# tejank10/AlphaGo.jl

Measured on AMD Instinct MI355X. Metric: self-play positions/sec (9x9, tower=10, 400 readouts), higher is better.
Workload: dtype f32

## Files before the change

### alphago.jl_amd/csrc/agz_nn.h

```cpp
#pragma once
#include <algorithm>
#include <cstdint>
#include <functional>
#include <memory>
#include <type_traits>
#include <vector>

#include "agz_common.h"

namespace agz {

constexpr int kC = 256;
constexpr int kCinStem = 17;
constexpr int kCinStemPad = 32;
constexpr int kWinoStages = 64, kWinoStemStages = 8;

struct ConvHost {
  int k = 3, cin = 0, cout = 0;
  std::vector<float> w, b, beta, gamma, mean, var;
  float eps = 1e-5f;
};
struct DenseHost {
  int in = 0, out = 0;
  std::vector<float> w, b;
// ... 55 lines not shown
    if (winograd_ == 0) return TowerForm::Direct;
    if (precision_ == 0 && winograd_ != 2 && wino4_applies(N_)) return TowerForm::Wino4;
    if (precision_ == 0 && winograd_ == 3 && wino_fusable(N_)) return TowerForm::Wino5;
    return tower_persistent_ && wino_fusable(N_) ? TowerForm::Wino3Persistent : TowerForm::Wino3;
  }

  float mfma_sustained_tflops(int millis, int mode = 0);
  void profile_enable(bool on);
  void profile_read(double* total_ms, double* total_flop, int64_t* launches);

  ConvHost* conv(int layer);
  const ConvHost* conv(int layer) const;
  DenseHost* dense(int layer);
  const DenseHost* dense(int layer) const;
  void sync_host() const;
  uint64_t param_version() const { return param_version_; }

  double flops_per_eval() const;
  double conv_flops_per_launch(int B) const { return 2.0 * B * P_ * 9.0 * kC * kC; }

 private:
  void pack();
  enum ImageId { kDirectStem, kDirectTower, kWinoStem, kWinoTower, kSplitStem, kSplitTower, kWino4Tower, kWino5Tower, kF16Tower, kImages };
  struct BuiltImage {
    const ImageFamily* family;
    bool stem;
    int which;
    bool (*needed)(const Net&);
    DevBuf<uint32_t> buf;
    uint64_t version = ~0ull;
  };
  static bool always(const Net&) { return true; }
  static bool with_tower(const Net& n) { return n.tower_ > 0; }
  static bool split_selected(const Net& n) { return n.tower_ > 0 && n.precision_ == 2; }
  template <TowerForm F> static bool form_is(const Net& n) { return n.tower_form() == F; }
  BuiltImage images_[kImages] = {{&kDirectImage, true, 0, always},
                                 {&kDirectImage, false, 0, with_tower},
                                 {&kWinoImage, true, 1, with_tower},
                                 {&kWinoImage, false, 1, with_tower},
                                 {&kWinoSplitImage, true, 4, split_selected},
                                 {&kWinoSplitImage, false, 4, split_selected},
                                 {&kWino4Image, false, 2, form_is<TowerForm::Wino4>},
                                 {&kWino5Image, false, 6, form_is<TowerForm::Wino5>},
                                 {&kConv16Image, false, 3, form_is<TowerForm::F16>}};
  uint64_t affines_version_ = ~0ull;
  int image_stages(const BuiltImage& im) const { return im.stem ? kWinoStemStages : kWinoStages; }
  template <class T>
  const T* image(ImageId id, int l = 0) const {
    const BuiltImage& im = images_[id];
    return reinterpret_cast<const T*>(im.buf.p + im.family->bytes(image_stages(im)) / 4 * l);
  }
  void stem(TowerForm form, const float* d_x32, const int* d_count, int bcap);
  void direct_tower(const int* d_count, int bcap);
  void f16_tower(const int* d_count, int bcap);
  void wino_tower(TowerForm form, const int* d_count, int bcap);
  void persistent_tower(const int* d_count, int bcap);
  struct LayerIO { const float *vin, *res; float *y, *vout; };
  LayerIO layer_io(int l, bool dense) const;
  void wino_layer(TowerForm form, int l, const LayerIO& io, const int* d_count, int bcap, hipStream_t st, int part = 0,
                  int parts = 1);
  template <class Layer> void run_chains(int chains, const Layer& layer);
  template <class Launch> void timed(int layers, const Launch& launch);

  int N_, P_, A_, tower_;
  hipStream_t stream_;
  ConvHost stem_, vconv_, pconv_;
  std::vector<ConvHost> tconv_;
  DenseHost vfc1_, vfc2_, pfc_;
  struct FluxSlot { int layer, kind; size_t off, n; };
  std::vector<FluxSlot> slots_;
  size_t flux_n_ = 0;
  DevBuf<float> d_flux_;
  mutable bool host_stale_ = false;
  uint64_t param_version_ = 0;
  void upload_slot(const FluxSlot& s);
  void upload_host_all();
  const float* host_slot(const FluxSlot& s) const;

  DevBuf<float> d_scale_, d_shift_;
  DevBuf<float> d_head_;
  const float *d_vfc1w_ = nullptr, *d_vfc1b_ = nullptr, *d_vfc2w_ = nullptr, *d_vfc2b_ = nullptr, *d_pfcw_ = nullptr,
              *d_pfcb_ = nullptr;
  int bcap_ = 0;
  DevBuf<float> d_a_, d_b_, d_t_, d_vh_, d_ph_;
  int winograd_ = 1;
  static constexpr int kMaxTowerStreams = 4;
  int tower_streams_ = 2;
  hipStream_t streamx_[kMaxTowerStreams - 1] = {nullptr, nullptr, nullptr};
  hipEvent_t ev_fork_ = nullptr, ev_join_[kMaxTowerStreams - 1] = {nullptr, nullptr, nullptr};
  DevBuf<float> d_scale_s_;
  DevBuf<float> d_vimg_, d_vimg2_;
  int precision_ = 0;
  DevBuf<uint16_t> d_ha_, d_hb_, d_ht_;
  bool tower_persistent_ = false;
  DevBuf<int> d_tower_sched_;
  DevBuf<char> d_tower_layers_;
  std::vector<char> tower_layers_host_;
  int32_t* tower_err_ = nullptr;
  std::vector<int> prof_mult_;
  bool prof_on_ = false;
  std::vector<hipEvent_t> prof_ev_;
  std::vector<int> prof_fwd_of_;
  int32_t* prof_counts_ = nullptr;
  int prof_n_ = 0, prof_fwd_ = 0;
  static constexpr int kProfMax = 4096;
};

class Trainer {
 public:
  Trainer(Net& net, hipStream_t s);
  ~Trainer();
  void step(const float* feats, const float* pi, const float* z, int B, bool is_device, float eta, float rho,
            float* losses_out);
  void reset();

 private:
  struct Param;
  void upload();
  void publish(long M);
  uint64_t uploaded_version_ = ~0ull;
  Net& net_;
  hipStream_t stream_;
  std::vector<std::unique_ptr<Param>> params_;
  bool have_vel_ = false;
  DevBuf<float> d_x32_, d_u_, d_o_, d_ga_, d_gb_, d_gc_, d_stats_, d_ones_, d_zero_, d_wd_, d_small_, d_in_, d_part_, d_wpart_;
  DevBuf<double> d_sums_;
  DevBuf<int> d_cnt_;
  DevBuf<unsigned char> d_opta_, d_optw_;
  int n_optw_ = 0;
};

void launch_conv3x3_direct_taps(const float* x, const float* wt, const float* ones, const float* zeros, const float* shift,
                                float* y, float* part, const int* d_count, int bcap, int N, int cin_pad, hipStream_t s);
int conv3x3_direct_blocks(int bcap, int N);
void launch_conv3x3_direct(const float* x, const float* wt, const float* scale, const float* shift, const float* res,
                           float* y, const int* d_count, int bcap, int N, int relu, int cin_pad, hipStream_t s);

size_t wino_v_floats(int bcap, int T);
long wino_blocks(int bcap, int T);
inline void wino_block_range(int blocks, int part, int parts, bool pairs, int& tb0, int& tb1) {
  AGZ_REQUIRE(parts >= 1 && part >= 0 && part < parts, AGZ_BAD_ARGUMENT, "tile-block range %d of %d", part, parts);
  int per = (blocks + parts - 1) / parts;
  if (pairs) per = (per + 1) & ~1;
  tb0 = std::min(blocks, part * per);
  tb1 = part + 1 == parts ? blocks : std::min(blocks, tb0 + per);
}
inline void wino_check_32bit(long blocks, int rows, int bcap, int N) {
  AGZ_REQUIRE((blocks + 1) * rows < (1L << 31) && (long)bcap * N * N * kC * 4 < (1L << 32), AGZ_BAD_ARGUMENT,
              "batch of %d positions at %dx%d: tile index / activation byte offset exceeds 32 bits", bcap, N, N);
}
void launch_wino_in(const float* x, float* vimg, const int* d_count, int bcap, int N, bool split, hipStream_t s,
                    int ns = kWinoStages, bool fixup = false);
void launch_wino_gemm(const float* vimg, const float* uimg, const float* scale, const float* shift, const float* res,
                      float* y, float* vnext, const int* d_count, int bcap, int N, int relu, bool split, hipStream_t s,
                      int ns = kWinoStages, int part = 0, int parts = 1);
bool wino_fusable(int N);
struct WinoTowerLayer {
  const float *v, *u, *scale, *shift, *res;
  float *y, *vnext;
  int mode, relu;
};
size_t wino_tower_sched_ints(int layers, int bcap, int N);
bool wino_tower_supported(hipStream_t s);
void launch_wino_tower(const void* d_layers, int layers, int* d_sched, const int* d_count, int bcap, int N, bool split, hipStream_t s);
constexpr int kWinoTowerErrWord = 8;
float wino_split_descale();

// ... 39 lines not shown
```

### alphago.jl_amd/csrc/agz_nn.hip

```cpp
#include "agz_nn.h"
#include "agz_pack.h"

#include <cmath>
#include <algorithm>
#include <cstring>

#include "../../include/agz_draws.h"

namespace agz {

typedef float f32x16 __attribute__((ext_vector_type(16)));


constexpr int BM = 128, BN = 128, BK = 32;
constexpr int LDS_STRIDE = BK + 4;

template <int CIN, bool TAPSPLIT = false>
__global__ __launch_bounds__(256, 2) void k_conv3x3_mfma(
    const float* __restrict__ x, const float* __restrict__ wt, const float* __restrict__ scale,
    const float* __restrict__ shift, const float* __restrict__ res, float* __restrict__ y,
    const int* __restrict__ d_count, int N, int relu, long ystride = 0) {
  constexpr int NCHUNK = 9 * CIN / BK;
  constexpr int CPT = CIN / BK;
  const int c_begin = TAPSPLIT ? (int)blockIdx.y * CPT : 0, c_end = TAPSPLIT ? c_begin + CPT : NCHUNK;
// ... 35 lines not shown
    const int tap_ = (c) / CPT, ci0_ = ((c) % CPT) * BK;          \
    const int da_ = tap_ % 3 - 1, db_ = tap_ / 3 - 1;             \
    const int aoff_ = ci0_ + c4 * 4, boff_ = (c) * BK;            \
    AGZ_LOADROW(0, da_, db_, aoff_, boff_)                        \
    AGZ_LOADROW(1, da_, db_, aoff_, boff_)                        \
    AGZ_LOADROW(2, da_, db_, aoff_, boff_)                        \
    AGZ_LOADROW(3, da_, db_, aoff_, boff_)                        \
  }
#define AGZ_STOREROW(buf, i)                                                                           \
  *reinterpret_cast<float4*>(&lds[buf][0][(lrow + 32 * i) * LDS_STRIDE + c4 * 4]) = ra##i;             \
  *reinterpret_cast<float4*>(&lds[buf][1][(lrow + 32 * i) * LDS_STRIDE + c4 * 4]) = rb##i;
#define AGZ_STORE_CHUNK(buf) { AGZ_STOREROW(buf, 0) AGZ_STOREROW(buf, 1) AGZ_STOREROW(buf, 2) AGZ_STOREROW(buf, 3) }

  const int lane = tid & 63, wave = tid >> 6;
  const int wr = wave >> 1, wc = wave & 1;
  const int l31 = lane & 31, hi = lane >> 5;

  f32x16 acc[2][2];
#pragma unroll
  for (int a = 0; a < 2; ++a)
#pragma unroll
    for (int b = 0; b < 2; ++b)
#pragma unroll
      for (int e = 0; e < 16; ++e) acc[a][b][e] = 0.f;

  AGZ_LOAD_CHUNK(c_begin)
  AGZ_STORE_CHUNK(0)
  __syncthreads();

  for (int c = c_begin; c < c_end; ++c) {
    const int buf = (c - c_begin) & 1;
    if (c + 1 < c_end) AGZ_LOAD_CHUNK(c + 1)
    const float* As = &lds[buf][0][(wr * 64 + l31) * LDS_STRIDE + hi * 4];
    const float* Bs = &lds[buf][1][(wc * 64 + l31) * LDS_STRIDE + hi * 4];
#pragma unroll
    for (int kk = 0; kk < BK / 8; ++kk) {
      const float4 a0 = *reinterpret_cast<const float4*>(As + kk * 8);
      const float4 a1 = *reinterpret_cast<const float4*>(As + 32 * LDS_STRIDE + kk * 8);
      const float4 b0 = *reinterpret_cast<const float4*>(Bs + kk * 8);
      const float4 b1 = *reinterpret_cast<const float4*>(Bs + 32 * LDS_STRIDE + kk * 8);
#define AGZ_MFMA4(f)                                                                          \
  acc[0][0] = __builtin_amdgcn_mfma_f32_32x32x2f32(a0.f, b0.f, acc[0][0], 0, 0, 0);             \
  acc[0][1] = __builtin_amdgcn_mfma_f32_32x32x2f32(a0.f, b1.f, acc[0][1], 0, 0, 0);             \
  acc[1][0] = __builtin_amdgcn_mfma_f32_32x32x2f32(a1.f, b0.f, acc[1][0], 0, 0, 0);             \
  acc[1][1] = __builtin_amdgcn_mfma_f32_32x32x2f32(a1.f, b1.f, acc[1][1], 0, 0, 0);
      AGZ_MFMA4(x) AGZ_MFMA4(y) AGZ_MFMA4(z) AGZ_MFMA4(w)
#undef AGZ_MFMA4
    }
    if (c + 1 < c_end) AGZ_STORE_CHUNK(buf ^ 1)
    __syncthreads();
  }

#undef AGZ_LOADROW
#undef AGZ_LOAD_CHUNK
#undef AGZ_STOREROW
#undef AGZ_STORE_CHUNK
#pragma unroll
  for (int tn = 0; tn < 2; ++tn) {
    const int n = n0 + wc * 64 + tn * 32 + l31;
    const float sc = scale[n], sh = shift[n];
#pragma unroll
    for (int tm = 0; tm < 2; ++tm) {
#pragma unroll
      for (int e = 0; e < 16; ++e) {
        const long m = m0 + wr * 64 + tm * 32 + (e & 3) + 8 * (e >> 2) + 4 * hi;
        if (m < M) {
          float v = acc[tm][tn][e] * sc + sh;
          if (res) v += res[m * kC + n];
          if (relu) v = fmaxf(v, 0.f);
          y[m * kC + n] = v;
        }
      }
    }
  }
}


__device__ __forceinline__ float wave_sum(float v) {
#pragma unroll
  for (int o = 32; o > 0; o >>= 1) v += __shfl_xor(v, o, 64);
  return v;
}

__global__ __launch_bounds__(256) void k_head_conv(const float* __restrict__ x, const float* __restrict__ hp,
                                                    float* __restrict__ vh, float* __restrict__ ph,
                                                    const int* __restrict__ d_count, int P) {
  const long M = (long)(*d_count) * P;
  const int lane = threadIdx.x & 63, wave = threadIdx.x >> 6;
  const float4 wv = *reinterpret_cast<const float4*>(hp + lane * 4);
  const float4 w0 = *reinterpret_cast<const float4*>(hp + 256 + lane * 4);
  const float4 w1 = *reinterpret_cast<const float4*>(hp + 512 + lane * 4);
  const float sv = hp[768], tv = hp[769], s0 = hp[770], t0 = hp[771], s1 = hp[772], t1 = hp[773];
  for (long m = (long)blockIdx.x * 4 + wave; m < M; m += (long)gridDim.x * 4) {
    const float4 xv = *reinterpret_cast<const float4*>(x + m * kC + lane * 4);
    float dv = xv.x * wv.x + xv.y * wv.y + xv.z * wv.z + xv.w * wv.w;
    float d0 = xv.x * w0.x + xv.y * w0.y + xv.z * w0.z + xv.w * w0.w;
    float d1 = xv.x * w1.x + xv.y * w1.y + xv.z * w1.z + xv.w * w1.w;
    dv = wave_sum(dv);
    d0 = wave_sum(d0);
    d1 = wave_sum(d1);
    if (lane == 0) {
      vh[m] = fmaxf(dv * sv + tv, 0.f);
      ph[m * 2 + 0] = fmaxf(d0 * s0 + t0, 0.f);
      ph[m * 2 + 1] = fmaxf(d1 * s1 + t1, 0.f);
    }
  }
}

__device__ float block_reduce(float v, bool is_max, float* red ) {
  const int lane = threadIdx.x & 63, wave = threadIdx.x >> 6;
#pragma unroll
  for (int o = 32; o > 0; o >>= 1) {
    const float t = __shfl_xor(v, o, 64);
    v = is_max ? fmaxf(v, t) : v + t;
  }
  __syncthreads();
  if (lane == 0) red[wave] = v;
  __syncthreads();
  float r = red[0];
#pragma unroll
  for (int w = 1; w < 4; ++w) r = is_max ? fmaxf(r, red[w]) : r + red[w];
  return r;
}

__global__ __launch_bounds__(256) void k_head_fc(
    const float* __restrict__ vh, const float* __restrict__ ph, const float* __restrict__ w1,
    const float* __restrict__ b1, const float* __restrict__ w2, const float* __restrict__ b2,
    const float* __restrict__ wp, const float* __restrict__ bp, float* __restrict__ pi,
    float* __restrict__ v, const int* __restrict__ d_count, int P, int A) {
  extern __shared__ __attribute__((aligned(16))) float sm[];
  float* vin = sm;
  float* pin = sm + P;
  float* logit = pin + 2 * P;
  float* red = logit + A;
  const int b = blockIdx.x;
  if (b >= *d_count) return;
  const int tid = threadIdx.x;
  for (int i = tid; i < P; i += 256) {
    vin[i] = vh[(long)b * P + i];
    pin[i] = ph[((long)b * P + i) * 2 + 0];
    pin[P + i] = ph[((long)b * P + i) * 2 + 1];
  }
  __syncthreads();
  float lmax = -INFINITY;
  for (int o = tid; o < A; o += 256) {
    float z = bp[o];
    for (int i = 0; i < 2 * P; ++i) z += wp[o + (long)A * i] * pin[i];
    logit[o] = z;
    lmax = fmaxf(lmax, z);
  }
  const float mx = block_reduce(lmax, true, red);
  float lsum = 0.f;
  for (int o = tid; o < A; o += 256) {
    const float e = expf(logit[o] - mx);
    logit[o] = e;
    lsum += e;
  }
  const float sum = block_reduce(lsum, false, red);
  for (int o = tid; o < A; o += 256) pi[(long)b * A + o] = logit[o] / sum;
  float h = b1[tid];
  for (int i = 0; i < P; ++i) h += w1[tid + 256 * i] * vin[i];
  h = fmaxf(h, 0.f);
  const float s = block_reduce(h * w2[tid], false, red);
  if (tid == 0) v[b] = tanhf(s + b2[0]);
}


__global__ __launch_bounds__(128) void k_feats_from_deltas(
    const int8_t* __restrict__ boards, const int8_t* __restrict__ deltas, const int32_t* __restrict__ ndeltas,
    const int8_t* __restrict__ to_play, int B, int N, float* __restrict__ x32, float* __restrict__ whcn) {
  const int b = blockIdx.x;
  if (b >= B) return;
  const int P = N * N;
  const int nd = ndeltas[b];
  const int tp = to_play[b];
  for (int p = threadIdx.x; p < P; p += blockDim.x) {
    int cur = boards[(long)b * P + p];
    float f[32];
#pragma unroll
    for (int k = 0; k < 8; ++k) {
      if (k >= 1 && k <= nd) cur -= deltas[((long)b * 7 + (k - 1)) * P + p];
      f[2 * k] = cur == tp ? 1.f : 0.f;
      f[2 * k + 1] = cur == -tp ? 1.f : 0.f;
    }
    f[16] = (float)tp;
#pragma unroll
    for (int c = 17; c < 32; ++c) f[c] = 0.f;
    if (x32) {
      float4* dst = reinterpret_cast<float4*>(x32 + ((long)b * P + p) * 32);
#pragma unroll
      for (int c = 0; c < 8; ++c) dst[c] = make_float4(f[4 * c], f[4 * c + 1], f[4 * c + 2], f[4 * c + 3]);
    }
    if (whcn) {
#pragma unroll
      for (int c = 0; c < 17; ++c) whcn[(long)P * (c + 17L * b) + p] = f[c];
    }
  }
}

__global__ __launch_bounds__(128) void k_whcn_to_x32(const float* __restrict__ whcn, int B, int P,
                                                      float* __restrict__ x32) {
  const int b = blockIdx.x;
  if (b >= B) return;
  for (int p = threadIdx.x; p < P; p += blockDim.x) {
    float* dst = x32 + ((long)b * P + p) * 32;
    for (int c = 0; c < 17; ++c) dst[c] = whcn[(long)P * (c + 17L * b) + p];
    for (int c = 17; c < 32; ++c) dst[c] = 0.f;
  }
}

void launch_features_from_deltas(const int8_t* d_boards, const int8_t* d_deltas, const int32_t* d_ndeltas,
                                 const int8_t* d_to_play, int B, int N, float* d_x32, float* d_whcn,
                                 hipStream_t stream) {
  if (B <= 0) return;
  hipLaunchKernelGGL(k_feats_from_deltas, dim3(B), dim3(128), 0, stream, d_boards, d_deltas, d_ndeltas,
                     d_to_play, B, N, d_x32, d_whcn);
  AGZ_HIP(hipGetLastError());
}

void launch_whcn_to_x32(const float* d_whcn, int B, int N, float* d_x32, hipStream_t stream) {
  if (B <= 0) return;
  hipLaunchKernelGGL(k_whcn_to_x32, dim3(B), dim3(128), 0, stream, d_whcn, B, N * N, d_x32);
  AGZ_HIP(hipGetLastError());
}


static void conv_init(ConvHost& c, int k, int cin, int cout) {
  c.k = k; c.cin = cin; c.cout = cout;
  c.w.assign((size_t)k * k * cin * cout, 0.f);
  c.b.assign(cout, 0.f);
  c.beta.assign(cout, 0.f);
  c.gamma.assign(cout, 1.f);
  c.mean.assign(cout, 0.f);
  c.var.assign(cout, 1.f);
  c.eps = 1e-5f;
}
static void dense_init(DenseHost& d, int in, int out) {
  d.in = in; d.out = out;
  d.w.assign((size_t)in * out, 0.f);
  d.b.assign(out, 0.f);
}

static std::vector<float>* conv_field(ConvHost* c, int kind);

Net::Net(int N, int tower, hipStream_t stream) : N_(N), P_(N * N), A_(N * N + 1), tower_(tower), stream_(stream) {
  conv_init(stem_, 3, kCinStem, kC);
  tconv_.resize(2 * tower);
// ... 236 lines not shown
    launched = true;
  }
  if (affines_version_ != param_version_) {
    d_scale_.ensure((size_t)L * kC);
    d_shift_.ensure((size_t)L * kC);
    d_scale_s_.ensure((size_t)L * kC);
    hipLaunchKernelGGL(k_bn_affine, dim3(1), dim3(256), 0, stream_, F + flux_offset(0, AGZ_K_BIAS), 0L, 1, kC, d_scale_.p, d_shift_.p,
                       d_scale_s_.p + (size_t)2 * tower_ * kC, wino_split_descale());
    if (tower_ > 0)
      hipLaunchKernelGGL(k_bn_affine, dim3(2 * tower_), dim3(256), 0, stream_, F + flux_offset(1, AGZ_K_BIAS), tstride(), 2 * tower_, kC,
                         d_scale_.p + kC, d_shift_.p + kC, d_scale_s_.p, wino_split_descale());
    d_head_.ensure(776);
    hipLaunchKernelGGL(k_pack_head, dim3(1), dim3(256), 0, stream_, F + flux_offset(AGZ_L_VALUE_CONV, AGZ_K_WEIGHT),
                       F + flux_offset(AGZ_L_POLICY_CONV, AGZ_K_WEIGHT), d_head_.p);
    d_vfc1w_ = F + flux_offset(AGZ_L_VALUE_FC1, AGZ_K_WEIGHT); d_vfc1b_ = F + flux_offset(AGZ_L_VALUE_FC1, AGZ_K_BIAS);
    d_vfc2w_ = F + flux_offset(AGZ_L_VALUE_FC2, AGZ_K_WEIGHT); d_vfc2b_ = F + flux_offset(AGZ_L_VALUE_FC2, AGZ_K_BIAS);
    d_pfcw_ = F + flux_offset(AGZ_L_POLICY_FC, AGZ_K_WEIGHT); d_pfcb_ = F + flux_offset(AGZ_L_POLICY_FC, AGZ_K_BIAS);
    affines_version_ = param_version_;
    launched = true;
  }
  if (launched) AGZ_HIP(hipGetLastError());
}

long Net::debug_pack_diff(int which) {
  pack();
  sync_host();
  if (which < 0 || which > 6) return -1;
  const int L = 1 + 2 * tower_;
  auto diff = [&](const auto* dev, const auto& host) {
    static_assert(sizeof(host[0]) == 4, "debug_pack_diff counts 32-bit words");
    auto got = host;
    download(got.data(), dev, got.size(), stream_);
    AGZ_HIP(hipStreamSynchronize(stream_));
    long bad = 0;
    for (size_t i = 0; i < got.size(); ++i) bad += std::memcmp(&got[i], &host[i], 4) != 0;
    return bad;
  };
  long bad = 0;
  for (const BuiltImage& im : images_) {
    if (im.which != which || !im.needed(*this)) continue;
    std::vector<uint32_t> img(im.family->bytes(image_stages(im)) / 4);
    for (int l = 0; l < (im.stem ? 1 : 2 * tower_); ++l) {
      im.family->host_pack(im.stem ? stem_ : tconv_[l], img.data(), image_stages(im));
      bad += diff(im.buf.p + img.size() * l, img);
    }
  }
  if (which == 4 && images_[kSplitTower].needed(*this)) {
    std::vector<float> sc((size_t)L * kC), tmp(kC);
    for (int l = 0; l <= 2 * tower_; ++l) {
      bn_affine(l < 2 * tower_ ? tconv_[l] : stem_, sc.data() + (size_t)l * kC, tmp.data());
      for (int o = 0; o < kC; ++o) sc[(size_t)l * kC + o] *= wino_split_descale();
    }
    bad += diff(d_scale_s_.p, sc);
  }
  if (which == 5) {
    std::vector<float> scale((size_t)L * kC), shift((size_t)L * kC);
    bn_affine(stem_, scale.data(), shift.data());
    for (int l = 0; l < 2 * tower_; ++l) bn_affine(tconv_[l], scale.data() + (size_t)(l + 1) * kC, shift.data() + (size_t)(l + 1) * kC);
    bad += diff(d_scale_.p, scale) + diff(d_shift_.p, shift);
    std::vector<float> hp(776, 0.f);
    for (int c = 0; c < kC; ++c) { hp[c] = vconv_.w[c]; hp[256 + c] = pconv_.w[c]; hp[512 + c] = pconv_.w[kC + c]; }
    float s[2], t[2];
    bn_affine(vconv_, s, t);
    hp[768] = s[0]; hp[769] = t[0];
    bn_affine(pconv_, s, t);
    hp[770] = s[0]; hp[771] = t[0]; hp[772] = s[1]; hp[773] = t[1];
    bad += diff(d_head_.p, hp);
  }
  return bad;
}

void Net::reserve(int bcap) {
  if (precision_ == 1 && tower_ > 0 && d_ha_.n < ((size_t)std::max(bcap, bcap_) * P_ + 256) * kC) {
    const size_t n = ((size_t)std::max(bcap, bcap_) * P_ + 256) * kC;
    d_ha_.alloc(n);
    d_hb_.alloc(n);
    d_ht_.alloc(n);
  }
  if (bcap <= bcap_) return;
  const size_t rows = (size_t)bcap * P_;
  d_a_.alloc(rows * kC);
  d_b_.alloc(rows * kC);
  d_t_.alloc(rows * kC);
  d_vh_.alloc(rows);
  d_ph_.alloc(rows * 2);
  if (tower_ > 0) {
    const size_t vf = std::max(wino_v_floats(bcap, (N_ + 2) / 3), wino4_applies(N_) ? wino4_v_floats(bcap, N_) : (size_t)0);
    d_vimg_.alloc(vf);
    d_vimg2_.alloc(vf);
  }
  bcap_ = bcap;
}

static inline int conv_grid(int bcap, int P) { return ceil_div((long)bcap * P, BM) * (kC / BN); }
int conv3x3_direct_blocks(int bcap, int N) { return conv_grid(bcap, N * N); }

void launch_conv3x3_direct(const float* x, const float* wt, const float* scale, const float* shift, const float* res,
                           float* y, const int* d_count, int bcap, int N, int relu, int cin_pad, hipStream_t s) {
  const int grid = conv_grid(bcap, N * N);
  if (cin_pad == kCinStemPad)
    hipLaunchKernelGGL((k_conv3x3_mfma<kCinStemPad>), dim3(grid), dim3(256), 0, s, x, wt, scale, shift, res, y, d_count, N, relu);
  else
    hipLaunchKernelGGL((k_conv3x3_mfma<kC>), dim3(grid), dim3(256), 0, s, x, wt, scale, shift, res, y, d_count, N, relu);
}

__global__ __launch_bounds__(256) void k_sum_taps(const float* __restrict__ part, long stride, const float* __restrict__ shift,
                                                   float* __restrict__ y, const int* __restrict__ d_count, int P) {
  const long n4 = (long)(*d_count) * P * (kC / 4);
  for (long i = (long)blockIdx.x * 256 + threadIdx.x; i < n4; i += (long)gridDim.x * 256) {
    float4 s = *reinterpret_cast<const float4*>(part + i * 4);
#pragma unroll
    for (int z = 1; z < 9; ++z) {
      const float4 v = *reinterpret_cast<const float4*>(part + z * stride + i * 4);
      s.x += v.x; s.y += v.y; s.z += v.z; s.w += v.w;
    }
    const float4 b = *reinterpret_cast<const float4*>(shift + (i * 4) % kC);
    *reinterpret_cast<float4*>(y + i * 4) = make_float4(s.x + b.x, s.y + b.y, s.z + b.z, s.w + b.w);
  }
}

void launch_conv3x3_direct_taps(const float* x, const float* wt, const float* ones, const float* zeros, const float* shift,
                                float* y, float* part, const int* d_count, int bcap, int N, int cin_pad, hipStream_t s) {
  const int grid = conv_grid(bcap, N * N);
  const long stride = (long)bcap * N * N * kC;
  if (cin_pad == kCinStemPad)
    hipLaunchKernelGGL((k_conv3x3_mfma<kCinStemPad, true>), dim3(grid, 9), dim3(256), 0, s, x, wt, ones, zeros,
                       (const float*)nullptr, part, d_count, N, 0, stride);
  else
    hipLaunchKernelGGL((k_conv3x3_mfma<kC, true>), dim3(grid, 9), dim3(256), 0, s, x, wt, ones, zeros, (const float*)nullptr,
                       part, d_count, N, 0, stride);
  const int g = (int)std::min<long>(((long)bcap * N * N * (kC / 4) + 255) / 256, 2048);
  hipLaunchKernelGGL(k_sum_taps, dim3(g), dim3(256), 0, s, (const float*)part, stride, shift, y, d_count, N * N);
}

template <class Launch> void Net::timed(int layers, const Launch& launch) {
  const bool p = prof_on_ && prof_n_ < kProfMax;
  if (p) (void)hipEventRecord(prof_ev_[2 * prof_n_], stream_);
  launch();
  if (p) {
    (void)hipEventRecord(prof_ev_[2 * prof_n_ + 1], stream_);
    prof_mult_[prof_n_] = layers;
    prof_fwd_of_[prof_n_++] = prof_fwd_;
  }
}

template <class Layer> void Net::run_chains(int chains, const Layer& layer) {
  const int nl = 2 * tower_;
  if (chains == 1) {
    for (int l = 0; l < nl; ++l) timed(1, [&] { layer(l, 0, stream_); });
    return;
  }
  if (!ev_fork_) AGZ_HIP(hipEventCreateWithFlags(&ev_fork_, hipEventDisableTiming));
  for (int i = 0; i + 1 < chains; ++i)
    if (!streamx_[i]) {
      AGZ_HIP(hipStreamCreateWithFlags(&streamx_[i], hipStreamNonBlocking));
      AGZ_HIP(hipEventCreateWithFlags(&ev_join_[i], hipEventDisableTiming));
    }
  auto join = [&] {
    for (int i = 0; i + 1 < chains; ++i) {
      (void)hipEventRecord(ev_join_[i], streamx_[i]);
      (void)hipStreamWaitEvent(stream_, ev_join_[i], 0);
    }
  };
  timed(nl, [&] {
    AGZ_HIP(hipEventRecord(ev_fork_, stream_));
    for (int i = 0; i + 1 < chains; ++i) AGZ_HIP(hipStreamWaitEvent(streamx_[i], ev_fork_, 0));
    try {
      for (int part = 0; part < chains; ++part)
// ... 79 lines not shown
  }
}

Net::LayerIO Net::layer_io(int l, bool dense) const {
  if (l % 2 == 0) return {d_vimg_.p, nullptr, dense ? d_t_.p : nullptr, d_vimg2_.p};
  const bool odd = (l / 2) % 2;
  return {d_vimg2_.p, odd ? d_b_.p : d_a_.p, odd ? d_a_.p : d_b_.p, l + 1 == 2 * tower_ ? nullptr : d_vimg_.p};
}

void Net::wino_layer(TowerForm form, int l, const LayerIO& io, const int* d_count, int bcap, hipStream_t st, int part, int parts) {
  const float* sc = d_scale_.p + (size_t)(l + 1) * kC;
  const float* sh = d_shift_.p + (size_t)(l + 1) * kC;
  if (form == TowerForm::Wino4) {
    launch_wino4_gemm(io.vin, image<float>(kWino4Tower, l), sc, sh, io.res, io.y, io.vout, d_count, bcap, N_, 1, st,
                      part, parts, io.y && !io.res && wino4_paired(N_));
    if (io.vout && !wino4_whole_boards(N_)) launch_wino4_in(io.y, io.vout, d_count, bcap, N_, st, true, part, parts);
  } else if (form == TowerForm::Wino5) {
    launch_wino5_gemm(io.vin, image<float>(kWino5Tower, l), sc, sh, io.res, io.y, io.vout, d_count, bcap, N_, 1, st,
                      part, parts);
  } else {
    const bool split = precision_ == 2;
    const float* u = image<float>(split ? kSplitTower : kWinoTower, l);
    launch_wino_gemm(io.vin, u, split ? d_scale_s_.p + (size_t)l * kC : sc, sh, io.res, io.y, io.vout, d_count, bcap, N_, 1, split,
                     st, kWinoStages, part, parts);
    if (io.vout && !wino_fusable(N_)) launch_wino_in(io.y, io.vout, d_count, bcap, N_, split, st, kWinoStages, true);
  }
}

void Net::wino_tower(TowerForm form, const int* d_count, int bcap) {
  const bool f44 = form == TowerForm::Wino4;
  const bool dense = f44 ? !wino4_whole_boards(N_) : !wino_fusable(N_);
  const int T = f44 ? (N_ + 3) / 4 : (N_ + 2) / 3;
  const int chains = dense && !f44 ? 1 : chain_count(tower_streams_, (long)bcap * T * T, f44 ? 64 : 63);
  run_chains(chains, [&](int l, int part, hipStream_t st) {
    wino_layer(form, l, layer_io(l, dense), d_count, bcap, st, part, chains);
  });
}

void Net::persistent_tower(const int* d_count, int bcap) {
  const bool split = precision_ == 2;
  const ImageId u = split ? kSplitTower : kWinoTower;
  const float* sc = split ? d_scale_s_.p : d_scale_.p + kC;
  const float* sh = d_shift_.p + kC;
  const int nl = 2 * tower_;
  std::vector<WinoTowerLayer> tab(nl);
  for (int l = 0; l < nl; ++l) {
    const LayerIO io = layer_io(l, false);
    tab[l] = {io.vin, image<float>(u, l), sc + (size_t)l * kC, sh + (size_t)l * kC, io.res, io.y, io.vout,
              (io.y ? 1 : 0) | (io.vout ? 2 : 0), 1};
  }
  const size_t tbytes = sizeof(WinoTowerLayer) * tab.size();
  if (tower_layers_host_.size() != tbytes || std::memcmp(tower_layers_host_.data(), tab.data(), tbytes) != 0) {
    AGZ_HIP(hipStreamSynchronize(stream_));
    tower_layers_host_.assign((const char*)tab.data(), (const char*)tab.data() + tbytes);
    d_tower_layers_.ensure(tbytes);
    AGZ_HIP(hipMemcpy(d_tower_layers_.p, tower_layers_host_.data(), tbytes, hipMemcpyHostToDevice));
  }
  d_tower_sched_.ensure(wino_tower_sched_ints(nl, bcap, N_));
  if (!tower_err_) {
    AGZ_HIP(hipHostMalloc((void**)&tower_err_, sizeof(int32_t), hipHostMallocDefault));
    *tower_err_ = 0;
  }
  timed(nl, [&] { launch_wino_tower(d_tower_layers_.p, nl, d_tower_sched_.p, d_count, bcap, N_, split, stream_); });
  (void)hipMemcpyAsync(tower_err_, d_tower_sched_.p + kWinoTowerErrWord, sizeof(int32_t), hipMemcpyDeviceToHost, stream_);
}

void Net::forward(const float* d_x32, const int* d_count, int bcap, float* d_pi, float* d_v) {
  check_async_error();
  TowerForm form = tower_form();
  if (form == TowerForm::Wino4) wino4_validate(bcap, N_);
  pack();
  reserve(bcap);
  if (prof_on_ && prof_fwd_ < kProfMax)
    (void)hipMemcpyAsync(&prof_counts_[prof_fwd_], d_count, sizeof(int32_t), hipMemcpyDeviceToHost, stream_);
  stem(form, d_x32, d_count, bcap);
  if (form == TowerForm::Wino3Persistent && !wino_tower_supported(stream_)) form = TowerForm::Wino3;
  switch (form) {
    case TowerForm::Direct: direct_tower(d_count, bcap); break;
    case TowerForm::F16: f16_tower(d_count, bcap); break;
    case TowerForm::Wino3Persistent: persistent_tower(d_count, bcap); break;
    default: wino_tower(form, d_count, bcap); break;
  }
  const float* x = form == TowerForm::F16 || tower_ % 2 ? d_b_.p : d_a_.p;
  const int hgrid = std::min(ceil_div((long)bcap * P_, 4), 256 * 16);
  hipLaunchKernelGGL(k_head_conv, dim3(hgrid), dim3(256), 0, stream_, x, d_head_.p, d_vh_.p, d_ph_.p, d_count, P_);
  const size_t smem = sizeof(float) * (size_t)(3 * P_ + A_ + 4);
  hipLaunchKernelGGL(k_head_fc, dim3(bcap), dim3(256), smem, stream_, (const float*)d_vh_.p,
                     (const float*)d_ph_.p, d_vfc1w_, d_vfc1b_, d_vfc2w_, d_vfc2b_, d_pfcw_,
                     d_pfcb_, d_pi, d_v, d_count, P_, A_);
  if (prof_on_ && prof_fwd_ < kProfMax) prof_fwd_++;
  AGZ_HIP(hipGetLastError());
}

__global__ __launch_bounds__(256) void k_mfma_f32_sustained(int iters, float* out) {
  typedef float f32x16 __attribute__((ext_vector_type(16)));
  f32x16 acc[8];
#pragma unroll
  for (int i = 0; i < 8; ++i)
#pragma unroll
    for (int e = 0; e < 16; ++e) acc[i][e] = 0.f;
  const float a = 1.f + threadIdx.x * 1e-6f, b = 0.5f;
  for (int it = 0; it < iters; ++it) {
#pragma unroll
    for (int i = 0; i < 8; ++i) acc[i] = __builtin_amdgcn_mfma_f32_32x32x2f32(a, b, acc[i], 0, 0, 0);
  }
  float s = 0.f;
#pragma unroll
  for (int i = 0; i < 8; ++i) s += acc[i][0] + acc[i][15];
  if (s == 123.456f) out[0] = s;
}

template <bool F16, bool DENSE>
__global__ __launch_bounds__(256) void k_mfma_sustained_data(int iters, float* out) {
  typedef float f32x16 __attribute__((ext_vector_type(16)));
  typedef _Float16 h8 __attribute__((ext_vector_type(8)));
  f32x16 acc[8];
#pragma unroll
  for (int i = 0; i < 8; ++i)
#pragma unroll
    for (int e = 0; e < 16; ++e) acc[i][e] = 0.f;
  unsigned st = 0x9e3779b9u * (threadIdx.x + 256u * blockIdx.x + 1u);
  auto rnd = [&]() { st = st * 1664525u + 1013904223u; return (float)(int)(st >> 8) * (1.0f / 8388608.0f) - 1.0f; };
  float a32[16], b32[16];
  h8 a16[16], b16[16];
#pragma unroll
  for (int k = 0; k < 16; ++k) {
    a32[k] = rnd(); b32[k] = DENSE ? rnd() : fmaxf(rnd(), 0.f) * 2.f;
#pragma unroll
    for (int e = 0; e < 8; ++e) {
      a16[k][e] = (_Float16)(0.06f * rnd());
      b16[k][e] = (_Float16)(DENSE ? rnd() : fmaxf(rnd(), 0.f) * 2.f);
    }
  }
  for (int it = 0; it < iters; it += 16) {
#pragma unroll
    for (int u = 0; u < 16; ++u)
#pragma unroll
      for (int i = 0; i < 8; ++i) {
        if (F16) acc[i] = __builtin_amdgcn_mfma_f32_32x32x16_f16(a16[(i + u) & 15], b16[(3 * i + 5 * u) & 15], acc[i], 0, 0, 0);
        else acc[i] = __builtin_amdgcn_mfma_f32_32x32x2f32(a32[(i + u) & 15], b32[(3 * i + 5 * u) & 15], acc[i], 0, 0, 0);
      }
  }
  float s = 0.f;
#pragma unroll
  for (int i = 0; i < 8; ++i) s += acc[i][0] + acc[i][15];
  if (s == 123.456f) out[0] = s;
}

float Net::mfma_sustained_tflops(int millis, int mode) {
  AGZ_REQUIRE(millis >= 50 && millis <= 5000, AGZ_BAD_ARGUMENT, "mfma_sustained_tflops: %d ms (50..5000)", millis);
  AGZ_REQUIRE(mode >= 0 && mode <= 4, AGZ_BAD_ARGUMENT, "mfma_sustained_tflops: mode %d", mode);
  const bool f16 = mode == 2 || mode == 4;
  DevBuf<float> out;
  out.alloc(16);
  hipEvent_t e0, e1;
  AGZ_HIP(hipEventCreate(&e0));
  AGZ_HIP(hipEventCreate(&e1));
  const int iters = f16 ? 20000 : 10000, grid = 1024;
  const double flop = (double)grid * 4 * iters * 8.0 * (f16 ? 32768.0 : 4096.0);
  std::vector<double> tf;
  double spent = 0.0;
  while (spent < millis) {
    AGZ_HIP(hipEventRecord(e0, stream_));
    if (mode == 0) hipLaunchKernelGGL(k_mfma_f32_sustained, dim3(grid), dim3(256), 0, stream_, iters, out.p);
    else if (mode == 1) hipLaunchKernelGGL((k_mfma_sustained_data<false, false>), dim3(grid), dim3(256), 0, stream_, iters, out.p);
    else if (mode == 2) hipLaunchKernelGGL((k_mfma_sustained_data<true, false>), dim3(grid), dim3(256), 0, stream_, iters, out.p);
    else if (mode == 3) hipLaunchKernelGGL((k_mfma_sustained_data<false, true>), dim3(grid), dim3(256), 0, stream_, iters, out.p);
    else hipLaunchKernelGGL((k_mfma_sustained_data<true, true>), dim3(grid), dim3(256), 0, stream_, iters, out.p);
    AGZ_HIP(hipEventRecord(e1, stream_));
    AGZ_HIP(hipEventSynchronize(e1));
    float ms = 0.f;
    AGZ_HIP(hipEventElapsedTime(&ms, e0, e1));
// ... 75 lines not shown
```

Measured before the change: 447.5.

## Fuse head conv and FC into one kernel processing eight boards per block

Merges the 1x1 head convolution and the value/policy fully connected layers into a single kernel, so the intermediate vh/ph buffers no longer go through global memory. Each block now handles eight boards, with per-board inputs interleaved in shared memory. Every weight loaded from wp and w1 is therefore reused across eight boards instead of being re-read per board. The trade-offs are fewer blocks (less parallelism for small batches), higher register pressure from the per-board arrays, and more shared memory per block.

Result: no change. 448.6, median of 3 (+0.2%).

```diff
diff --git a/alphago.jl_amd/csrc/agz_nn.h b/alphago.jl_amd/csrc/agz_nn.h
--- a/alphago.jl_amd/csrc/agz_nn.h
+++ b/alphago.jl_amd/csrc/agz_nn.h
@@ -161,7 +161,7 @@
   const float *d_vfc1w_ = nullptr, *d_vfc1b_ = nullptr, *d_vfc2w_ = nullptr, *d_vfc2b_ = nullptr, *d_pfcw_ = nullptr,
               *d_pfcb_ = nullptr;
   int bcap_ = 0;
-  DevBuf<float> d_a_, d_b_, d_t_, d_vh_, d_ph_;
+  DevBuf<float> d_a_, d_b_, d_t_;
   int winograd_ = 1;
   static constexpr int kMaxTowerStreams = 4;
   int tower_streams_ = 2;
diff --git a/alphago.jl_amd/csrc/agz_nn.hip b/alphago.jl_amd/csrc/agz_nn.hip
--- a/alphago.jl_amd/csrc/agz_nn.hip
+++ b/alphago.jl_amd/csrc/agz_nn.hip
@@ -141,31 +141,6 @@
   return v;
 }
 
-__global__ __launch_bounds__(256) void k_head_conv(const float* __restrict__ x, const float* __restrict__ hp,
-                                                    float* __restrict__ vh, float* __restrict__ ph,
-                                                    const int* __restrict__ d_count, int P) {
-  const long M = (long)(*d_count) * P;
-  const int lane = threadIdx.x & 63, wave = threadIdx.x >> 6;
-  const float4 wv = *reinterpret_cast<const float4*>(hp + lane * 4);
-  const float4 w0 = *reinterpret_cast<const float4*>(hp + 256 + lane * 4);
-  const float4 w1 = *reinterpret_cast<const float4*>(hp + 512 + lane * 4);
-  const float sv = hp[768], tv = hp[769], s0 = hp[770], t0 = hp[771], s1 = hp[772], t1 = hp[773];
-  for (long m = (long)blockIdx.x * 4 + wave; m < M; m += (long)gridDim.x * 4) {
-    const float4 xv = *reinterpret_cast<const float4*>(x + m * kC + lane * 4);
-    float dv = xv.x * wv.x + xv.y * wv.y + xv.z * wv.z + xv.w * wv.w;
-    float d0 = xv.x * w0.x + xv.y * w0.y + xv.z * w0.z + xv.w * w0.w;
-    float d1 = xv.x * w1.x + xv.y * w1.y + xv.z * w1.z + xv.w * w1.w;
-    dv = wave_sum(dv);
-    d0 = wave_sum(d0);
-    d1 = wave_sum(d1);
-    if (lane == 0) {
-      vh[m] = fmaxf(dv * sv + tv, 0.f);
-      ph[m * 2 + 0] = fmaxf(d0 * s0 + t0, 0.f);
-      ph[m * 2 + 1] = fmaxf(d1 * s1 + t1, 0.f);
-    }
-  }
-}
-
 __device__ float block_reduce(float v, bool is_max, float* red ) {
   const int lane = threadIdx.x & 63, wave = threadIdx.x >> 6;
 #pragma unroll
@@ -182,46 +157,112 @@
   return r;
 }
 
-__global__ __launch_bounds__(256) void k_head_fc(
-    const float* __restrict__ vh, const float* __restrict__ ph, const float* __restrict__ w1,
+constexpr int kHeadBoards = 8;
+inline size_t head_smem_bytes(int P, int A) { return sizeof(float) * ((size_t)kHeadBoards * (3 * P + A) + 4); }
+template <int G>
+__global__ __launch_bounds__(256) void k_heads(
+    const float* __restrict__ x, const float* __restrict__ hp, const float* __restrict__ w1,
     const float* __restrict__ b1, const float* __restrict__ w2, const float* __restrict__ b2,
     const float* __restrict__ wp, const float* __restrict__ bp, float* __restrict__ pi,
     float* __restrict__ v, const int* __restrict__ d_count, int P, int A) {
+  static_assert(G % 4 == 0, "the positions of an input point are read as float4s");
   extern __shared__ __attribute__((aligned(16))) float sm[];
   float* vin = sm;
-  float* pin = sm + P;
-  float* logit = pin + 2 * P;
-  float* red = logit + A;
-  const int b = blockIdx.x;
-  if (b >= *d_count) return;
-  const int tid = threadIdx.x;
-  for (int i = tid; i < P; i += 256) {
-    vin[i] = vh[(long)b * P + i];
-    pin[i] = ph[((long)b * P + i) * 2 + 0];
-    pin[P + i] = ph[((long)b * P + i) * 2 + 1];
+  float* pin = sm + G * P;
+  float* logit = pin + 2 * G * P;
+  float* red = logit + G * A;
+  const int count = *d_count;
+  const int b0 = blockIdx.x * G;
+  if (b0 >= count) return;
+  const int nb = min(G, count - b0);
+  const int tid = threadIdx.x, lane = tid & 63, wave = tid >> 6;
+  {
+    const float4 wv = *reinterpret_cast<const float4*>(hp + lane * 4);
+    const float4 w0 = *reinterpret_cast<const float4*>(hp + 256 + lane * 4);
+    const float4 wq = *reinterpret_cast<const float4*>(hp + 512 + lane * 4);
+    const float sv = hp[768], tv = hp[769], s0 = hp[770], t0 = hp[771], s1 = hp[772], t1 = hp[773];
+    const float* xb = x + (long)b0 * P * kC + lane * 4;
+    const int np = nb * P;
+    for (int q0 = wave; q0 < G * P; q0 += 16) {
+      float4 xv[4];
+#pragma unroll
+      for (int u = 0; u < 4; ++u) {
+        const int q = q0 + 4 * u;
+        xv[u] = q < np ? *reinterpret_cast<const float4*>(xb + (long)q * kC) : make_float4(0.f, 0.f, 0.f, 0.f);
+      }
+#pragma unroll
+      for (int u = 0; u < 4; ++u) {
+        const int q = q0 + 4 * u;
+        float dv = xv[u].x * wv.x + xv[u].y * wv.y + xv[u].z * wv.z + xv[u].w * wv.w;
+        float d0 = xv[u].x * w0.x + xv[u].y * w0.y + xv[u].z * w0.z + xv[u].w * w0.w;
+        float d1 = xv[u].x * wq.x + xv[u].y * wq.y + xv[u].z * wq.z + xv[u].w * wq.w;
+        dv = wave_sum(dv);
+        d0 = wave_sum(d0);
+        d1 = wave_sum(d1);
+        if (lane == 0 && q < G * P) {
+          const int g = q / P, i = q - g * P;
+          vin[i * G + g] = fmaxf(dv * sv + tv, 0.f);
+          pin[i * G + g] = fmaxf(d0 * s0 + t0, 0.f);
+          pin[(P + i) * G + g] = fmaxf(d1 * s1 + t1, 0.f);
+        }
+      }
+    }
   }
   __syncthreads();
-  float lmax = -INFINITY;
+  typedef float f32x4 __attribute__((ext_vector_type(4)));
+  float lmax[G];
+#pragma unroll
+  for (int g = 0; g < G; ++g) lmax[g] = -INFINITY;
   for (int o = tid; o < A; o += 256) {
-    float z = bp[o];
-    for (int i = 0; i < 2 * P; ++i) z += wp[o + (long)A * i] * pin[i];
-    logit[o] = z;
-    lmax = fmaxf(lmax, z);
-  }
-  const float mx = block_reduce(lmax, true, red);
-  float lsum = 0.f;
-  for (int o = tid; o < A; o += 256) {
-    const float e = expf(logit[o] - mx);
-    logit[o] = e;
-    lsum += e;
-  }
-  const float sum = block_reduce(lsum, false, red);
-  for (int o = tid; o < A; o += 256) pi[(long)b * A + o] = logit[o] / sum;
-  float h = b1[tid];
-  for (int i = 0; i < P; ++i) h += w1[tid + 256 * i] * vin[i];
-  h = fmaxf(h, 0.f);
-  const float s = block_reduce(h * w2[tid], false, red);
-  if (tid == 0) v[b] = tanhf(s + b2[0]);
+    float z[G];
+#pragma unroll
+    for (int g = 0; g < G; ++g) z[g] = bp[o];
+#pragma unroll 8
+    for (int i = 0; i < 2 * P; ++i) {
+      const float w = wp[o + (long)A * i];
+#pragma unroll
+      for (int g4 = 0; g4 < G; g4 += 4) {
+        const f32x4 in = *reinterpret_cast<const f32x4*>(pin + i * G + g4);
+#pragma unroll
+        for (int e = 0; e < 4; ++e) z[g4 + e] += w * in[e];
+      }
+    }
+#pragma unroll
+    for (int g = 0; g < G; ++g) {
+      logit[g * A + o] = z[g];
+      lmax[g] = fmaxf(lmax[g], z[g]);
+    }
+  }
+  float h[G];
+#pragma unroll
+  for (int g = 0; g < G; ++g) h[g] = b1[tid];
+#pragma unroll 8
+  for (int i = 0; i < P; ++i) {
+    const float w = w1[tid + 256 * i];
+#pragma unroll
+    for (int g4 = 0; g4 < G; g4 += 4) {
+      const f32x4 in = *reinterpret_cast<const f32x4*>(vin + i * G + g4);
+#pragma unroll
+      for (int e = 0; e < 4; ++e) h[g4 + e] += w * in[e];
+    }
+  }
+  const float w2t = w2[tid], b2v = b2[0];
+#pragma unroll
+  for (int g = 0; g < G; ++g) {
+    if (g >= nb) break;
+    float* lg = logit + g * A;
+    const float mx = block_reduce(lmax[g], true, red);
+    float lsum = 0.f;
+    for (int o = tid; o < A; o += 256) {
+      const float e = expf(lg[o] - mx);
+      lg[o] = e;
+      lsum += e;
+    }
+    const float sum = block_reduce(lsum, false, red);
+    for (int o = tid; o < A; o += 256) pi[(long)(b0 + g) * A + o] = lg[o] / sum;
+    const float s = block_reduce(fmaxf(h[g], 0.f) * w2t, false, red);
+    if (tid == 0) v[b0 + g] = tanhf(s + b2v);
+  }
 }
 
 
@@ -624,8 +665,6 @@
   d_a_.alloc(rows * kC);
   d_b_.alloc(rows * kC);
   d_t_.alloc(rows * kC);
-  d_vh_.alloc(rows);
-  d_ph_.alloc(rows * 2);
   if (tower_ > 0) {
     const size_t vf = std::max(wino_v_floats(bcap, (N_ + 2) / 3), wino4_applies(N_) ? wino4_v_floats(bcap, N_) : (size_t)0);
     d_vimg_.alloc(vf);
@@ -871,12 +910,8 @@
     default: wino_tower(form, d_count, bcap); break;
   }
   const float* x = form == TowerForm::F16 || tower_ % 2 ? d_b_.p : d_a_.p;
-  const int hgrid = std::min(ceil_div((long)bcap * P_, 4), 256 * 16);
-  hipLaunchKernelGGL(k_head_conv, dim3(hgrid), dim3(256), 0, stream_, x, d_head_.p, d_vh_.p, d_ph_.p, d_count, P_);
-  const size_t smem = sizeof(float) * (size_t)(3 * P_ + A_ + 4);
-  hipLaunchKernelGGL(k_head_fc, dim3(bcap), dim3(256), smem, stream_, (const float*)d_vh_.p,
-                     (const float*)d_ph_.p, d_vfc1w_, d_vfc1b_, d_vfc2w_, d_vfc2b_, d_pfcw_,
-                     d_pfcb_, d_pi, d_v, d_count, P_, A_);
+  hipLaunchKernelGGL(k_heads<kHeadBoards>, dim3(ceil_div(bcap, kHeadBoards)), dim3(256), head_smem_bytes(P_, A_), stream_, x,
+                     (const float*)d_head_.p, d_vfc1w_, d_vfc1b_, d_vfc2w_, d_vfc2b_, d_pfcw_, d_pfcb_, d_pi, d_v, d_count, P_, A_);
   if (prof_on_ && prof_fwd_ < kProfMax) prof_fwd_++;
   AGZ_HIP(hipGetLastError());
 }
```
